# land1725/albedo

Measured on AMD Instinct MI355X. Metric: implicit-ALS interactions/sec per sweep at rank 128 (1/8 GPU); top-30 recs users/sec, higher is better.
Workload: dtype fp32 (split-fp16x3 MFMA build, fp32 accumulate; fp64 Gram/eigenbasis)

## Files before the change

albedo_amd/csrc/als_engine.cpp:

```cpp
#include <hip/hip_runtime.h>
#include <rccl/rccl.h>

#include <algorithm>
#include <chrono>
#include <thread>
#include <cmath>
#include <cstdlib>
#include <functional>
#include <mutex>
#include <cstring>
#include <numeric>
#include <string>
#include <vector>

#include "albedo_als.h"
#include "engine.h"
#include "host_math.h"
#include "kernels.h"

using namespace albedo;

namespace {

thread_local std::string g_err;
// ... 9 lines not shown
#define NCCLCHK(x)                                                                                 \
  do {                                                                                             \
    ncclResult_t r_ = (x);                                                                         \
    if (r_ != ncclSuccess) return fail(ALS_E_RCCL, std::string("RCCL error: ") + ncclGetErrorString(r_) + " in " #x); \
  } while (0)

int albedo::set_device(als_ctx* c) {
  HIPCHK(hipSetDevice(c->dev));
  return ALS_OK;
}

hipError_t albedo::copy_st(const als_ctx* c, void* dst, const void* src, size_t bytes, hipMemcpyKind kind) {
  if (bytes == 0) return hipSuccess;
  const hipError_t e = hipMemcpyAsync(dst, src, bytes, kind, c->st);
  return e != hipSuccess ? e : hipStreamSynchronize(c->st);
}

namespace {

hipError_t fill_st(const als_ctx* c, void* dst, int v, size_t bytes) {
  if (bytes == 0) return hipSuccess;
  const hipError_t e = hipMemsetAsync(dst, v, bytes, c->st);
  return e != hipSuccess ? e : hipStreamSynchronize(c->st);
}

int drain(als_ctx* c) {
  if (c->st2) HIPCHK(hipStreamSynchronize(c->st2));
  if (c->st) HIPCHK(hipStreamSynchronize(c->st));
  return ALS_OK;
}

int validate(const als_params* p) {
  auto bad = [](const char* name, double v) {
    char buf[160];
    snprintf(buf, sizeof buf, "als parameter %s given invalid value %g.", name, v);
    return fail(ALS_E_INVALID_ARGUMENT, buf);
  };
  if (p->rank < 1) return bad("rank", p->rank);
  if (p->max_iter < 0) return bad("maxIter", p->max_iter);
  if (!(p->reg_param >= 0)) return bad("regParam", p->reg_param);
  if (!(p->alpha >= 0)) return bad("alpha", p->alpha);
  if (p->num_user_blocks < 1) return bad("numUserBlocks", p->num_user_blocks);
  if (p->num_item_blocks < 1) return bad("numItemBlocks", p->num_item_blocks);
  if (padded_rank(p->rank) == 0)
    return fail(ALS_E_UNSUPPORTED, "rank " + std::to_string(p->rank) + " exceeds the compiled maximum (256)");
  return ALS_OK;
}

int64_t light_limit(const als_ctx* c) {
  if (c->p.light_max_degree >= 0) return std::min<int64_t>(c->p.light_max_degree, c->KP == 128 ? 96 : 64);
  return c->KP >= 128 ? 64 : 32;
}

int bucket_of(int64_t d, int64_t lmax) {
  if (d <= lmax) {
    if (d <= 16) return B_L16;
    if (d <= 32) return B_L32;
    return d <= 64 ? B_L64 : B_L96;
  }
  return B_HEAVY;
}

int allreduce_G(als_ctx* c) {
  const int64_t n = (int64_t)c->KP * c->KP;
  if (c->world == 1) return ALS_OK;
  if (c->comm) {
    NCCLCHK(ncclAllReduce(c->d_G.p, c->d_G.p, n, ncclDouble, ncclSum, c->comm, c->st));
    return ALS_OK;
  }
  std::vector<double> h(n);
  HIPCHK(hipMemcpyAsync(h.data(), c->d_G.p, n * 8, hipMemcpyDeviceToHost, c->st));
  HIPCHK(hipStreamSynchronize(c->st));
  if (c->h_allreduce(c->h_user, h.data(), n) != 0) return fail(ALS_E_RCCL, "host all-reduce callback failed");
  HIPCHK(hipMemcpyAsync(c->d_G.p, h.data(), n * 8, hipMemcpyHostToDevice, c->st));
  HIPCHK(hipStreamSynchronize(c->st));
  return ALS_OK;
}

int allgather_rows(als_ctx* c, float* buf, int64_t rows_per_rank, hipStream_t s) {
  if (c->world == 1) return ALS_OK;
  const int64_t per = rows_per_rank * c->KP;
  if (c->comm) {
    NCCLCHK(ncclAllGather(buf + (int64_t)c->rank * per, buf, per, ncclFloat, c->comm, s));
    return ALS_OK;
  }
  std::vector<float> h((size_t)per * c->world);
  HIPCHK(hipMemcpyAsync(h.data() + (size_t)c->rank * per, buf + (int64_t)c->rank * per, per * 4,
                        hipMemcpyDeviceToHost, s));
  HIPCHK(hipStreamSynchronize(s));
  if (c->h_allgather(c->h_user, h.data(), per) != 0) return fail(ALS_E_RCCL, "host all-gather callback failed");
  HIPCHK(hipMemcpyAsync(buf, h.data(), h.size() * 4, hipMemcpyHostToDevice, s));
  HIPCHK(hipStreamSynchronize(s));
  return ALS_OK;
}

}

int albedo::allgather_host(als_ctx* c, float* buf, int64_t n) {
  if (c->world == 1) return ALS_OK;
  if (c->comm) {
    DevBuf d;
    HIPCHK(d.ensure((size_t)n * c->world * 4));
    float* dp = d.as<float>();
    HIPCHK(hipMemcpyAsync(dp + (int64_t)c->rank * n, buf + (int64_t)c->rank * n, n * 4, hipMemcpyHostToDevice, c->st));
    NCCLCHK(ncclAllGather(dp + (int64_t)c->rank * n, dp, n, ncclFloat, c->comm, c->st));
    HIPCHK(hipMemcpyAsync(buf, dp, (size_t)n * c->world * 4, hipMemcpyDeviceToHost, c->st));
    HIPCHK(hipStreamSynchronize(c->st));
    return ALS_OK;
  }
  if (c->h_allgather(c->h_user, buf, n) != 0) return fail(ALS_E_RCCL, "host all-gather callback failed");
  return ALS_OK;
}

namespace {

int gather_chunks(als_ctx* c, const Side& S, const float* own, float* full, int q0, int q1, hipStream_t s) {
  const int64_t per = S.chpad * c->KP;
  for (int q = q0; q < q1; ++q) {
    float* base = full + (int64_t)q * c->world * per;
    HIPCHK(hipMemcpyAsync(base + (int64_t)c->rank * per, own + (int64_t)q * per, per * 4, hipMemcpyDeviceToDevice, s));
    TRYC(allgather_rows(c, base, S.chpad, s));
  }
  return ALS_OK;
}

int split_chunk_len() {
  const char* e = std::getenv("ALBEDO_SPLIT_CHUNK");
  if (e && *e) return std::max(0, std::atoi(e));
  return 8192;
}

constexpr int BATCH_SLOTS[5] = {16, 8, 4, 2, 1};
constexpr int BATCH_MIN_SLOTS = 8;
int nnls_min_slots() {
  const char* e = std::getenv("ALBEDO_NNLS_MIN_SLOTS");
  const int v = e && *e ? std::atoi(e) : BATCH_MIN_SLOTS;
  return (v == 16 || v == 8 || v == 4 || v == 2 || v == 1) ? v : BATCH_MIN_SLOTS;
}
int64_t nnls_batch_rows_limit(const als_ctx* c, int v) {
  if (BATCH_SLOTS[v] < nnls_min_slots()) return 0;
  return std::min<int64_t>(nnls_batch_max_degree(c->KP, BATCH_SLOTS[v]), light_limit(c));
}

int gather_chunk_count() { return 4; }

bool use_wave_kernel(const als_ctx* c);

int factor_buffers(als_ctx* c);

int rank_layout(als_ctx* c) {
  TRYC(drain(c));
  const int64_t lmax = light_limit(c);
  c->split_len = split_chunk_len();
  for (int side = 0; side < 2; ++side) {
    Side& S = c->s[side];
    std::vector<int32_t> rows[NBUCKET];
    for (int b = 0; b < NBUCKET; ++b) S.bnnz[b] = 0;
    for (int64_t r = 0; r < S.own_n; ++r) {
      const int b = bucket_of(S.h_deg[r], lmax);
      rows[b].push_back((int32_t)r);
      S.bnnz[b] += S.h_deg[r];
    }
    std::stable_sort(rows[B_HEAVY].begin(), rows[B_HEAVY].end(),
                     [&](int32_t a, int32_t b) { return S.h_deg[a] > S.h_deg[b]; });
    S.n_batch = S.n_batch_nnz = 0;
    for (int v = 0; v < 6; ++v) S.bat_off[v] = 0;
    if (c->p.nonnegative) {
      for (int b = 0; b < B_HEAVY; ++b)
        std::stable_sort(rows[b].begin(), rows[b].end(), [&](int32_t x, int32_t y) { return S.h_deg[x] < S.h_deg[y]; });
      int64_t pos = 0;
      std::vector<int32_t> light;
      for (int b = 0; b < B_HEAVY; ++b) light.insert(light.end(), rows[b].begin(), rows[b].end());
      for (int v = 0; v < 5; ++v) {
        const int64_t dl = nnls_batch_rows_limit(c, v);
        while (pos < (int64_t)light.size() && S.h_deg[light[pos]] <= dl) S.n_batch_nnz += S.h_deg[light[pos++]];
        S.bat_off[v + 1] = pos;
      }
      S.n_batch = pos;
    }
    const int nsolve = (c->world > 1 && !c->p.nonnegative) ? S.nch : 1;
    S.nsolve = nsolve;
    auto chunk_of = [&](int32_t r) { return nsolve == 1 ? 0 : (int)std::min<int64_t>(r / S.chpad, nsolve - 1); };
    std::vector<int32_t> all;
    all.reserve(S.own_n);
    for (int b = 0; b < NBUCKET; ++b) {
      S.boff[b] = (int64_t)all.size();
      const bool pairs = b == B_L16;
      std::stable_sort(rows[b].begin(), rows[b].end(), [&](int32_t x, int32_t y) {
        const int cx = chunk_of(x), cy = chunk_of(y);
        if (cx != cy || !pairs) return cx < cy;
        return (S.h_deg[x] <= 8) > (S.h_deg[y] <= 8);
      });
      int64_t p = 0;
      for (int q = 0; q <= nsolve; ++q) {
        while (q < nsolve && p < (int64_t)rows[b].size() && chunk_of(rows[b][p]) < q) ++p;
        S.cb[b][q] = S.boff[b] + (q == nsolve ? (int64_t)rows[b].size() : p);
      }
      if (pairs)
        for (int q = 0; q < nsolve; ++q) {
          int64_t k = 0;
          for (int64_t i = S.cb[b][q] - S.boff[b]; i < S.cb[b][q + 1] - S.boff[b] && S.h_deg[rows[b][i]] <= 8; ++i) ++k;
          S.c8[q] = k;
        }
      all.insert(all.end(), rows[b].begin(), rows[b].end());
    }
    S.boff[NBUCKET] = (int64_t)all.size();
    HIPCHK(S.d_rows.ensure(all.size() * 4));
    HIPCHK(copy_st(c, S.d_rows.p, all.data(), all.size() * 4, hipMemcpyHostToDevice));
    HIPCHK(S.d_desc.ensure(all.size() * 16));
    HIPCHK(launch_row_desc(S.d_rows.as<int32_t>(), (int64_t)all.size(), S.d_ptr.as<int64_t>(), S.d_desc.as<int32_t>(), c->st));
    HIPCHK(hipStreamSynchronize(c->st));
    const int64_t CH = c->split_len;
// ... 187 lines not shown
  S.orig_valid = false;
  S.full_valid = false;
  return ALS_OK;
}

int spark_init(als_ctx* c) {
  int64_t su, si;
  spark_side_seeds(c->p.seed, &su, &si);
  for (int side = 0; side < 2; ++side) {
    Side& S = c->s[side];
    if (S.has_factors) continue;
    std::vector<float> f((size_t)S.n * c->p.rank);
    spark_initialize(S.ids.data(), S.n, c->p.rank, side == ALS_USER ? su : si,
                     side == ALS_USER ? c->p.num_user_blocks : c->p.num_item_blocks, f.data(), c->p.rank);
    TRYC(upload_factors(c, side, f.data(), c->p.rank));
  }
  return ALS_OK;
}

std::string err_paths(int err) {
  std::string r;
  const std::pair<int, const char*> names[] = {{ALBEDO_EF_LIGHT16, "light16"}, {ALBEDO_EF_LIGHT_REG, "light-d16"},
                                               {ALBEDO_EF_LIGHT_ACC, "light"}, {ALBEDO_EF_WAVE, "wave"},
                                               {ALBEDO_EF_HEAVY, "heavy"}};
  for (const auto& n : names)
    if (err & n.first) r += std::string(r.empty() ? ": " : ",") + n.second;
  return r;
}

}

float albedo::event_ms(hipEvent_t a, hipEvent_t b) {
  float ms = 0.f;
  (void)hipEventElapsedTime(&ms, a, b);
  return ms;
}

namespace {

int column_scales(als_ctx* c, const Side& S, const Side& T, bool have_max = false) {
  const float cmax = c->p.implicit_prefs ? (float)c->p.alpha * T.vmax : 1.0f;
  HIPCHK(launch_colscale(c->KP, S.d_Z.as<float>(), S.prows(), cmax, c->d_csmax.as<unsigned>(),
                         c->d_cs.as<float>(), c->st, have_max));
  return ALS_OK;
}

int heavy_launches(als_ctx* c, const Side& T, SolveArgs a, int64_t h0, int64_t hn, bool nnls, int q = 0);
bool use_wave_kernel(const als_ctx* c);

bool rotate_bf_on(const als_ctx* c) { return c->KP == 128; }

bool presplit_wanted(const als_ctx* c, const Side& T, float* sw) {
  const bool uniform = !c->p.implicit_prefs || (T.vmin == T.vmax && T.vmax > 0.f);
  if (!uniform || !use_wave_kernel(c) || T.boff[NBUCKET] == T.boff[B_HEAVY]) return false;
  const float cw = c->p.implicit_prefs ? (float)c->p.alpha * T.vmax : 1.0f;
  if (!(cw > 0.f)) return false;
  *sw = std::sqrt(cw);
  return true;
}

int presplit(als_ctx* c, const Side& S, const Side& T, const void** zhl, float* wsc, float* inv_sw,
             bool split_done = false) {
  *zhl = nullptr;
  float sw = 1.f;
  if (!presplit_wanted(c, T, &sw)) return ALS_OK;
  const float cw = c->p.implicit_prefs ? (float)c->p.alpha * T.vmax : 1.0f;
  HIPCHK(c->d_Zhl.ensure((size_t)(S.prows() + 1) * c->KP * 4));
  if (!split_done)
    HIPCHK(launch_presplit(c->KP, S.d_Z.as<float>(), S.prows(), c->d_cs.as<float>(), sw, c->d_Zhl.p, c->st));
  const double wmax = c->p.implicit_prefs ? 1.0 + (double)cw : (double)T.vmax;
  int e = 0;
  std::frexp(wmax > 0.0 ? wmax : 1.0, &e);
  *wsc = (float)std::ldexp(1.0, std::max(-60, std::min(60, 13 - e)));
  *inv_sw = 1.0f / sw;
  *zhl = c->d_Zhl.p;
  return ALS_OK;
}

int half_sweep_nnls(als_ctx* c, int t) {
  const int sidx = 1 - t;
  Side& S = c->s[sidx];
  Side& T = c->s[t];
  const int KP = c->KP, k = c->p.rank;
  hipStream_t st = c->st;
  hipEvent_t* ev = c->ev;
  const int ngt = nnls_gtile_floats(KP);
  std::vector<float> gt(ngt, 0.f);
  float gscale = 1.0f;
  if (c->p.implicit_prefs) {
    HIPCHK(launch_gram(KP, S.d_X.as<float>(), S.own_n, c->slab.as<double>(), c->slab_blocks, c->d_G.as<double>(), st));
    TRYC(allreduce_G(c));
    std::vector<double> Gf((size_t)KP * KP);
    HIPCHK(hipMemcpyAsync(Gf.data(), c->d_G.p, Gf.size() * 8, hipMemcpyDeviceToHost, st));
    HIPCHK(hipMemcpyAsync(S.d_Gk.p, c->d_G.p, (size_t)KP * KP * 8, hipMemcpyDeviceToDevice, st));
    HIPCHK(hipMemcpyAsync(S.d_GB.p, S.d_B.p, (size_t)KP * KP * 8, hipMemcpyDeviceToDevice, st));
    HIPCHK(hipStreamSynchronize(st));
    S.has_gram = true;
    for (int i = 0; i < KP; ++i)
      for (int j = 0; j < 16 * ((i >> 4) + 1); ++j) gt[nnls_gtile_index(i, j)] = (float)Gf[(size_t)i * KP + j];
    double gmax = 0.0;
    for (double v : Gf) gmax = std::max(gmax, std::fabs(v));
    if (gmax > 0.0) {
      int ex = 0;
      (void)std::frexp(gmax, &ex);
      gscale = (float)std::ldexp(1.0, std::max(-120, std::min(120, 15 - ex)));
    }
  }
// ... 194 lines not shown
    }
    HIPCHK(hipEventRecord(ev[2], st));
    const float* Xs = multi ? S.d_Xfull.as<float>() : S.d_X.as<float>();
    const int64_t ns = multi ? S.prows() : S.own_n;
    if (rotate_bf_on(c) && !singular) {
      TRYC(column_scales(c, S, T, true));
      cs_done = true;
      float sw = 1.f;
      split_done = presplit_wanted(c, T, &sw);
      if (split_done) HIPCHK(c->d_Zhl.ensure((size_t)(S.prows() + 1) * KP * 4));
      HIPCHK(c->d_Pf.ensure((size_t)rotate_bf_pfrag_bytes(KP)));
      HIPCHK(launch_rotate_bf(KP, Xs, c->d_P.as<float>(), c->d_Pf.p, S.d_Z.as<float>(), ns, c->d_cs.as<float>(), sw,
                              split_done ? c->d_Zhl.p : nullptr, S.prows(), c->n_cu, st));
    } else {
      HIPCHK(hipMemsetAsync(c->d_csmax.p, 0, KP * sizeof(unsigned), st));
      HIPCHK(launch_rotate(KP, Xs, c->d_P.as<float>(), S.d_Z.as<float>(), ns, st, c->d_csmax.as<unsigned>()));
      have_cmax = true;
    }
  } else {
    HIPCHK(hipEventRecord(ev[1], st));
    HIPCHK(hipMemsetAsync(c->d_lam.p, 0, KP * 4, st));
    HIPCHK(hipMemcpyAsync(T.d_B.p, S.d_B.p, (size_t)KP * KP * 8, hipMemcpyDeviceToDevice, st));
    if (c->p.reg_param == 0.0) force_heavy = true;
    HIPCHK(hipEventRecord(ev[2], st));
    if (multi) HIPCHK(hipMemcpyAsync(S.d_Z.p, S.d_Xfull.p, (size_t)S.prows() * KP * 4, hipMemcpyDeviceToDevice, st));
    else HIPCHK(hipMemcpyAsync(S.d_Z.p, S.d_X.p, (size_t)S.own_n * KP * 4, hipMemcpyDeviceToDevice, st));
  }
  HIPCHK(hipEventRecord(ev[3], st));
  if (!cs_done) TRYC(column_scales(c, S, T, have_cmax));
  const void* zhl = nullptr;
  float wsc = 1.f, inv_sw = 1.f;
  TRYC(presplit(c, S, T, &zhl, &wsc, &inv_sw, split_done));
  HIPCHK(hipEventRecord(ev[4], st));
  HIPCHK(hipMemsetAsync(c->d_err.p, 0, 4, st));
  SolveArgs a{};
  a.Zhl = zhl;
  a.zero_row = S.prows();
  a.wsc = wsc;
  a.inv_sw = inv_sw;
  a.Z = S.d_Z.as<float>();
  a.ptr = T.d_ptr.as<int64_t>();
  a.col = T.d_col.as<int32_t>();
  a.val = T.d_val.as<float>();
  a.lam = c->d_lam.as<float>();
  a.X = T.d_X.as<float>();
  a.kreal = k;
  a.implicit = c->p.implicit_prefs;
  a.alpha = (float)c->p.alpha;
  a.reg = (float)c->p.reg_param;
  a.err = c->d_err.as<int>();
  a.colscale = c->d_cs.as<float>();
  a.n_cu = c->n_cu;
  const int32_t* rows = T.d_rows.as<int32_t>();
  static const int Dof[B_HEAVY] = {16, 32, 64, 96};
  T.stats[0] = T.stats[1] = T.stats[2] = T.stats[3] = 0;
  for (int b = 0; b < B_HEAVY; ++b) {
    T.stats[force_heavy ? 2 : 0] += T.boff[b + 1] - T.boff[b];
    T.stats[force_heavy ? 3 : 1] += T.bnnz[b];
  }
  T.stats[2] += T.boff[B_HEAVY + 1] - T.boff[B_HEAVY];
  T.stats[3] += T.bnnz[B_HEAVY];
  for (int q = 0; q < T.nsolve; ++q) {
    for (int b = 0; b < B_HEAVY; ++b) {
      a.rows = rows + T.cb[b][q];
      a.desc = T.d_desc.as<int32_t>() + 4 * T.cb[b][q];
      a.n_rows = T.cb[b][q + 1] - T.cb[b][q];
      if (force_heavy && use_wave_kernel(c)) HIPCHK(launch_solve_wave(KP, a, st));
      else if (force_heavy) HIPCHK(launch_solve_heavy(KP, a, st));
      else if (b == B_L16) {
        SolveArgs p8 = a, p16 = a;
        p8.n_rows = T.c8[q];
        p16.rows += T.c8[q];
        p16.desc += 4 * T.c8[q];
        p16.n_rows -= T.c8[q];
        HIPCHK(launch_solve_light16(KP, p8, st, true));
        HIPCHK(launch_solve_light16(KP, p16, st, false));
      } else HIPCHK(launch_solve_light(KP, Dof[b], a, st));
    }
    if (T.nsolve == 1) HIPCHK(hipEventRecord(ev[5], st));
    TRYC(heavy_launches(c, T, a, T.cb[B_HEAVY][q], T.cb[B_HEAVY][q + 1] - T.cb[B_HEAVY][q], false, q));
    if (multi) {
      HIPCHK(hipEventRecord(c->evc[q], st));
      HIPCHK(hipStreamWaitEvent(c->st2, c->evc[q], 0));
      TRYC(gather_chunks(c, T, T.d_X.as<float>(), T.d_Xfull.as<float>(), q, q + 1, c->st2));
    }
  }
  if (T.nsolve > 1) HIPCHK(hipEventRecord(ev[5], st));
  if (multi) {
    if (T.nsolve == 1) TRYC(gather_chunks(c, T, T.d_X.as<float>(), T.d_Xfull.as<float>(), 0, T.nch, c->st2));
    HIPCHK(hipEventRecord(c->evc[8], c->st2));
  }
  HIPCHK(hipEventRecord(ev[6], st));
  int err = 0, sweeps = 0;
  HIPCHK(hipMemcpyAsync(&err, c->d_err.p, 4, hipMemcpyDeviceToHost, st));
  if (c->p.implicit_prefs) HIPCHK(hipMemcpyAsync(&sweeps, eig_sweeps(c->d_eig.as<double>(), KP), 4, hipMemcpyDeviceToHost, st));
  HIPCHK(hipStreamSynchronize(st));
  T.solver[0] = sweeps == EIG_NOT_FINITE ? 0 : (sweeps < 0 ? -sweeps - 1 : sweeps);
  T.solver[1] = T.solver[2] = T.solver[3] = 0;
  T.t[ALS_T_GRAM] = event_ms(ev[0], ev[1]);
  T.t[ALS_T_EIG] = event_ms(ev[1], ev[2]);
  T.t[ALS_T_ROTATE] = event_ms(ev[2], ev[3]);
  T.t[ALS_T_COMM] = event_ms(ev[3], ev[4]);
  if (T.nsolve > 1) {
    T.t[ALS_T_SOLVE_LIGHT] = 0.0;
    T.t[ALS_T_SOLVE_HEAVY] = event_ms(ev[4], ev[5]);
  } else {
    T.t[ALS_T_SOLVE_LIGHT] = event_ms(ev[4], ev[5]);
    T.t[ALS_T_SOLVE_HEAVY] = event_ms(ev[5], ev[6]);
  }
  T.t[ALS_T_HALF_TOTAL] = event_ms(ev[0], ev[6]);
  if (sweeps == EIG_NOT_FINITE)
    return fail(ALS_E_NOT_POSITIVE_DEFINITE,
                std::string("the ") + (t == ALS_USER ? "item" : "user") +
                    " Gram matrix is not finite (NaN or Inf in the source factors, or row norms past fp32): "
                    "the eigensolver did not converge");
  if (sweeps < 0)
    return fail(ALS_E_NOT_POSITIVE_DEFINITE, "eigensolver did not converge (device Jacobi: " +
                                                 std::to_string(-sweeps - 1) + " sweeps without meeting the tolerance)");
  if (err & 3)
    return fail(ALS_E_NOT_POSITIVE_DEFINITE,
                "LAPACK.dppsv-equivalent Cholesky met a non-positive pivot because A is not positive "
                "definite. Is A derived from a singular matrix (e.g. collinear column values)? (flags " +
                    std::to_string(err) + err_paths(err) + ", " + std::to_string(sweeps) + " eigensolver sweeps, " +
                    (t == ALS_USER ? "user" : "item") + " half)" +
                    failure_diag(c, S, T, c->p.implicit_prefs ? (multi ? S.prows() : S.own_n) : S.own_n, zhl));
  T.has_factors = true;
  T.orig_valid = false;
  T.full_valid = multi;
  return ALS_OK;
}

}
// ... 95 lines not shown
    return fail(ALS_E_HIP, "failed to create a HIP stream");
  }
  for (auto& e : c->ev) (void)hipEventCreate(&e);
  for (auto& e : c->evt) (void)hipEventCreate(&e);
  for (auto& e : c->evc) (void)hipEventCreateWithFlags(&e, hipEventDisableTiming);
  if (hipStreamCreateWithFlags(&c->st2, hipStreamNonBlocking) != hipSuccess) {
    delete c;
    return fail(ALS_E_HIP, "failed to create a HIP stream");
  }
  *out = c;
  return ALS_OK;
}

int als_create(const als_params* p, als_ctx** out) {
  if (!p || !out) return fail(ALS_E_INVALID_ARGUMENT, "null argument");
  *out = nullptr;
  TRYC(validate(p));
  return ctx_common(p, out);
}

int als_set_params(als_ctx* c, const als_params* p) {
  if (!c || !p) return fail(ALS_E_INVALID_ARGUMENT, "null argument");
  if (c->model_only) return fail(ALS_E_STATE, "als_set_params on a model-only context");
  if (c->parent) return fail(ALS_E_STATE, "als_set_params on a fork (fork the parent again instead)");
  {
    std::lock_guard<std::mutex> lk(g_fork_mu);
    if (c->forks > 0) return fail(ALS_E_STATE, "als_set_params while forks view this context's layout");
  }
  TRYC(validate(p));
  TRYC(set_device(c));
  const int dev = c->dev;
  c->p = *p;
  c->p.device = dev;
  c->KP = padded_rank(p->rank);
  if (c->has_ratings) TRYC(rank_layout(c));
  return ALS_OK;
}

int als_fork(als_ctx* parent, const als_params* p, als_ctx** out) {
  if (!parent || !p || !out) return fail(ALS_E_INVALID_ARGUMENT, "null argument");
  *out = nullptr;
  if (!parent->has_ratings || parent->model_only) return fail(ALS_E_STATE, "als_fork needs a context holding ratings");
  if (parent->world > 1) return fail(ALS_E_UNSUPPORTED, "als_fork of a sharded (multi-rank) context");
  TRYC(validate(p));
  if (p->rank != parent->p.rank || p->nonnegative != parent->p.nonnegative ||
      p->light_max_degree != parent->p.light_max_degree)
    return fail(ALS_E_INVALID_ARGUMENT, "a fork keeps its parent's rank, nonnegative and light_max_degree");
  als_params q = *p;
  q.device = parent->dev;
  als_ctx* c = nullptr;
  TRYC(ctx_common(&q, &c));
  c->nnz = parent->nnz;
  c->split_len = parent->split_len;
  for (int side = 0; side < 2; ++side) {
    Side& S = c->s[side];
    const Side& P = parent->s[side];
    S.n = P.n;
    S.ids = P.ids;
    S.starts = P.starts;
    S.maxrows = P.maxrows;
    S.nch = P.nch;
    S.world = P.world;
    S.chpad = P.chpad;
    S.own0 = P.own0;
    S.own_n = P.own_n;
    S.own_nnz = P.own_nnz;
    S.h_deg = P.h_deg;
    S.vmax = P.vmax;
    S.vmin = P.vmin;
    S.d_ptr.share(P.d_ptr);
    S.d_col.share(P.d_col);
    S.d_val.share(P.d_val);
    S.d_rows.share(P.d_rows);
    S.d_desc.share(P.d_desc);
    S.d_chunk_row.share(P.d_chunk_row);
    S.d_chunk_idx.share(P.d_chunk_idx);
    S.d_slot0.share(P.d_slot0);
    std::memcpy(S.boff, P.boff, sizeof S.boff);
    std::memcpy(S.bnnz, P.bnnz, sizeof S.bnnz);
    S.n_split = P.n_split;
    S.n_chunks = P.n_chunks;
    S.n_batch = P.n_batch;
    S.n_batch_nnz = P.n_batch_nnz;
    std::memcpy(S.bat_off, P.bat_off, sizeof S.bat_off);
    S.nsolve = P.nsolve;
    std::memcpy(S.cb, P.cb, sizeof S.cb);
    std::memcpy(S.c8, P.c8, sizeof S.c8);
    std::memcpy(S.split_n, P.split_n, sizeof S.split_n);
    std::memcpy(S.ck_off, P.ck_off, sizeof S.ck_off);
    std::memcpy(S.sl_off, P.sl_off, sizeof S.sl_off);
  }
  {
    std::lock_guard<std::mutex> lk(g_fork_mu);
    ++parent->forks;
  }
  c->parent = parent;
  c->has_ratings = true;
  if (int rc = set_device(c); rc != ALS_OK || (rc = factor_buffers(c)) != ALS_OK) {
    const std::string msg = g_err;
    als_destroy(c);
    return fail(rc, msg);
  }
  *out = c;
  return ALS_OK;
}

// ... 495 lines not shown
```

albedo_amd/csrc/als_kernels.hip:

```cpp
#include <hip/hip_runtime.h>
#include <cmath>
#include <cstdlib>
#include <cstdint>
#include <type_traits>
#include <algorithm>
#include <utility>
#include "kernels.h"
#include "device_common.h"
#include "wave_chol.h"
#include "nnls_common.h"
#include "split_rec.h"

namespace albedo {

inline SolveArgs chunk_args(const SolveArgs& a, int64_t r0, int threads, int rec_floats) {
  SolveArgs b = a;
  b.rows = a.rows + r0;
  b.n_rows = std::min<int64_t>(a.n_rows - r0, max_rows_per_launch(threads));
  if (a.prebuilt) b.prebuilt = a.prebuilt + (size_t)r0 * rec_floats;
  return b;
}

#ifdef ALBEDO_HEAVY_TIMING
__device__ unsigned long long albedo_heavy_ts[64][48];
// ... 489 lines not shown
  f32x4 xa[NK][2], xb[NK][2];
  if (t < ntile) xload(t, xa);
  if (t + tstep < ntile) xload(t + tstep, xb);
  for (; t < ntile; t += 2 * tstep) {
    tile(t, xa, t + 2 * tstep);
    if (t + tstep >= ntile) break;
    tile(t + tstep, xb, t + 3 * tstep);
  }
}

hipError_t launch_rotate_bf(int KP, const float* X, const float* P, void* Pf, float* Z, int64_t n, const float* cs, float sw,
                            void* Zhl, int64_t zrow, int n_cu, hipStream_t s) {
  if (KP != 128) return hipErrorInvalidValue;
  rotate_pfrag_kernel<<<(KP * KP + 255) / 256, 256, 0, s>>>(P, reinterpret_cast<__bf16*>(Pf), KP);
  if (n <= 0) return hipGetLastError();
  const size_t lds = (size_t)KP * KP * 3 * 2 + (size_t)RBF_WAVES * 16 * RBF_TS * 4 + (size_t)KP * 4;
  static const hipError_t attr = allow_lds(rotate_bf_kernel<128>, lds);
  if (attr != hipSuccess) return attr;
  const int64_t tiles = (n + 15) / 16;
  int64_t blocks = (tiles + RBF_WAVES - 1) / RBF_WAVES;
  if (blocks > n_cu) blocks = n_cu;
  rotate_bf_kernel<128><<<(int)blocks, 64 * RBF_WAVES, lds, s>>>(X, reinterpret_cast<const __bf16*>(Pf), Z, n, cs, sw,
                                                                 reinterpret_cast<_Float16*>(Zhl), zrow);
  return hipGetLastError();
}
int rotate_bf_pfrag_bytes(int KP) { return KP * KP * 3 * 2; }

hipError_t launch_rotate(int KP, const float* X, const float* M, float* Z, int64_t n, hipStream_t s, unsigned* cmax) {
  if (n <= 0) return hipSuccess;
  int64_t blocks = (n + 16 * ROT_WAVES - 1) / (16 * ROT_WAVES);
  if (blocks > 1024) blocks = 1024;
  const int nth = 64 * ROT_WAVES;
  if (KP == 64) {
    const size_t lds = (size_t)64 * 68 * 4;
    rotate_kernel<64><<<(int)blocks, nth, lds, s>>>(X, M, Z, n, cmax);
  } else if (KP == 128) {
    const size_t lds = (size_t)128 * 132 * 4;
    static const hipError_t attr = allow_lds(rotate_kernel<128>, lds);
    if (attr != hipSuccess) return attr;
    rotate_kernel<128><<<(int)blocks, nth, lds, s>>>(X, M, Z, n, cmax);
  } else if (KP == 256) {
    const size_t lds = (size_t)256 * (rotate_cols<256>() + 4) * 4;
    static const hipError_t attr = allow_lds(rotate_kernel<256>, lds);
    if (attr != hipSuccess) return attr;
    rotate_kernel<256><<<dim3((int)blocks, 256 / rotate_cols<256>()), nth, lds, s>>>(X, M, Z, n, cmax);
  } else return hipErrorInvalidValue;
  return hipGetLastError();
}

__host__ __device__ constexpr int light_wave_lds(int D) { return D == 16 ? D * (D + 1) / 2 + 64 : wchol_scratch_floats(D / 16); }

template <int KP, int D>
constexpr int light_occupancy() {
  return D > 64 ? 2 : (D == 16 && KP <= 128) ? 6 : (KP == 128 && D == 32) ? 3 : (KP <= 128) ? 4 : 2;
}

template <int KP, int D>
constexpr bool light_keepz() { return D <= 32 && D * KP <= 4096; }
template <int KP, int D>
constexpr bool light_split_s() { return D >= 64 || light_keepz<KP, D>(); }

template <int KP, int D>
__device__ __forceinline__ void light_row(const SolveArgs& a, int j, int d, float r, int colE, float r2, int colE2,
                                          const float (&lamv)[KP / 64], const float (&icsv)[KP / 64], float* smem,
                                          int wave) {
  constexpr int NB = D / 16, NT = NB * (NB + 1) / 2, TRI = light_wave_lds(D), NHC = KP / 64;
  constexpr bool TWO = D > 64;
  const int lane = threadIdx.x & 63, g = lane >> 4, i16 = lane & 15;
  float* Ks = smem + wave * TRI;
  float ce = 0.f, we = 0.f, ce2 = 0.f, we2 = 0.f;
  if (lane < d) rating_weights(r, a.implicit, a.alpha, ce, we);
  if (TWO && 64 + lane < d) rating_weights(r2, a.implicit, a.alpha, ce2, we2);
  const bool valid = lane < d && ce > 0.f;
  const bool valid2 = TWO && 64 + lane < d && ce2 > 0.f;
  const int npos = a.implicit ? __popcll(__ballot(lane < d && r > 0.f)) + (TWO ? __popcll(__ballot(64 + lane < d && r2 > 0.f)) : 0)
                              : d;
  const float lamn = a.reg * (float)npos;

  int colB[NB];
  bool vB[NB];
#pragma unroll
  for (int I = 0; I < NB; ++I) {
    colB[I] = __shfl(I < 4 ? colE : colE2, 16 * (I & 3) + i16);
    vB[I] = __shfl((int)(I < 4 ? valid : valid2), 16 * (I & 3) + i16) != 0;
  }
  constexpr int NC = KP / 16;
  constexpr bool KEEPZ = light_keepz<KP, D>();
  f32x4 zf[KEEPZ ? NB : 1][KEEPZ ? NC : 1];
  if constexpr (KEEPZ) {
#pragma unroll
    for (int I = 0; I < NB; ++I)
#pragma unroll
      for (int c = 0; c < NC; ++c) zf[I][c] = vB[I] ? ld4(a.Z + (int64_t)colB[I] * KP + 16 * c + 4 * g) : zero4();
  }
  constexpr bool PUSHG = !KEEPZ && D >= 64;
  constexpr int LATE = (KP == 128 && D == 64) ? 2 : 0;
  f32x4 zr0[PUSHG ? NB : 1], zr1[PUSHG ? NB : 1];
  const float* zpB[PUSHG ? NB : 1];
  if constexpr (PUSHG) {
#pragma unroll
    for (int I = 0; I < NB; ++I) {
      zpB[I] = a.Z + (vB[I] ? (int64_t)colB[I] : a.zero_row) * KP + 8 * g;
      zr0[I] = ld4(zpB[I]);
      zr1[I] = ld4(zpB[I] + 4);
    }
  }
  f32x4 acc[NT];
#pragma unroll
  for (int t = 0; t < NT; ++t) acc[t] = zero4();
  float* sdl = smem + 4 * TRI + wave * KP;
  bool bad = false;
#pragma unroll
  for (int h = 0; h < NHC; ++h) {
    const int cc = lane + 64 * h;
    const float dd = lamv[h] + lamn;
    if (cc < a.kreal && !(dd > 0.f)) bad = true;
    sdl[cc] = (cc < a.kreal && dd > 0.f) ? frsq(dd) : 0.f;
  }
  WAVE_LDS_SYNC();
  if constexpr (light_split_s<KP, D>()) {
    float bnd = 0.f;
#pragma unroll
    for (int h = 0; h < NHC; ++h) {
      const int cc = lane + 64 * h;
      bnd = fmaxf(bnd, sdl[cc] * icsv[h]);
    }
    bnd = wave_max_dpp(bnd);
    int ex = 0;
    frexpf(bnd * 8192.f, &ex);
    const float sc = ldexpf(1.f, 13 - ex), usc = ldexpf(1.f, 2 * (ex - 13));
    constexpr int NQ = KP / 32;
#pragma unroll
    for (int q = 0; q < NQ; ++q) {
      if constexpr (PUSHG) {
        __builtin_amdgcn_sched_barrier(0);
        if (q > 0) {
#pragma unroll
          for (int I = NB - LATE; I < NB; ++I) {
            zr0[I] = ld4(zpB[I] + 32 * q);
            zr1[I] = ld4(zpB[I] + 32 * q + 4);
          }
          __builtin_amdgcn_sched_barrier(0);
        }
      }
      const f32x4 s0 = KEEPZ ? ld4(sdl + 32 * q + 4 * g) : ld4(sdl + 32 * q + 8 * g);
      const f32x4 s1 = KEEPZ ? ld4(sdl + 32 * q + 16 + 4 * g) : ld4(sdl + 32 * q + 8 * g + 4);
      f16x8 zh[NB], zl[NB];
#pragma unroll
      for (int I = 0; I < NB; ++I) {
// ... 191 lines not shown
    for (int h = 0; h < NHC; ++h) sd[h] = sdl[NHC * lane + h];
    *reinterpret_cast<xvec*>(a.X + (int64_t)j * KP + NHC * lane) = xacc * (sd * sd);
  }
}

template <int KP, int D>
__global__ __launch_bounds__(256, (light_occupancy<KP, D>())) void solve_light_kernel(SolveArgs a) {
  extern __shared__ __attribute__((aligned(16))) float smem[];
  const int lane = threadIdx.x & 63;
  const int wave = __builtin_amdgcn_readfirstlane(threadIdx.x >> 6);
  const int64_t ridx = (int64_t)blockIdx.x * 4 + wave;
  if (ridx >= a.n_rows) return;
  float lamv[KP / 64], icsv[KP / 64];
#pragma unroll
  for (int h = 0; h < KP / 64; ++h) {
    lamv[h] = a.lam[lane + 64 * h];
    icsv[h] = light_split_s<KP, D>() ? a.colscale[KP + lane + 64 * h] : 0.f;
  }
  typedef __attribute__((address_space(4))) const int cint;
  cint* q = (cint*)(a.desc) + 4 * ridx;
  const int j = q[0], d = q[3];
  const int64_t p0 = (int64_t)(uint32_t)q[1] | ((int64_t)q[2] << 32);
  float r = 0.f, r2 = 0.f;
  int colE = 0, colE2 = 0;
  if (lane < d) {
    r = a.val[p0 + lane];
    colE = a.col[p0 + lane];
  }
  if (D > 64 && 64 + lane < d) {
    r2 = a.val[p0 + 64 + lane];
    colE2 = a.col[p0 + 64 + lane];
  }
  light_row<KP, D>(a, j, d, r, colE, r2, colE2, lamv, icsv, smem, wave);
}

hipError_t launch_solve_light(int KP, int D, const SolveArgs& a0, hipStream_t s) {
  if (a0.n_rows <= 0) return hipSuccess;
  if (!a0.desc) return hipErrorInvalidValue;
  if (a0.n_rows > max_rows_per_launch(64)) {
    for (int64_t r0 = 0; r0 < a0.n_rows; r0 += max_rows_per_launch(64)) {
      SolveArgs b = chunk_args(a0, r0, 64, 0);
      b.desc = a0.desc + 4 * r0;
      const hipError_t e = launch_solve_light(KP, D, b, s);
      if (e != hipSuccess) return e;
    }
    return hipSuccess;
  }
  const SolveArgs& a = a0;
  const size_t lds = ((size_t)4 * light_wave_lds(D) + (size_t)4 * KP) * sizeof(float);
  const int blocks = (int)((a.n_rows + 3) / 4);
#define LIGHT(kp, dd) \
  if (KP == kp && D == dd) { solve_light_kernel<kp, dd><<<blocks, 256, lds, s>>>(a); return hipGetLastError(); }
  LIGHT(64, 16) LIGHT(64, 32) LIGHT(64, 64) LIGHT(128, 16) LIGHT(128, 32) LIGHT(128, 64)
  LIGHT(256, 16) LIGHT(256, 32) LIGHT(256, 64) LIGHT(128, 96)
#undef LIGHT
  return hipErrorInvalidValue;
}



template <int KP>
struct Heavy {
  static constexpr int NW = KP >= 256 ? 16 : 4, NTH = 64 * NW, NQ = KP / 16;
  static constexpr int SPS = KP >= 256 ? 64 : 32;
  static constexpr int NU = SPS / 8;
  static constexpr int CS = 2 * SPS;
  static constexpr int IMG = KP * CS;
  static constexpr int NCH = KP / 4, NSG = NTH / NCH, NST = SPS / NSG;
  static constexpr bool PERM = KP != 256;
  static constexpr int SWZ = NU == 4 ? 3 : 5;
  static constexpr int GS = KP == 64 ? 2 : 4, NG = NQ / GS;
  static constexpr int NTL = NQ * (NQ + 1) / 2;
  static constexpr int TILES = NTL * HT_SZ, STAGE = IMG;
  static constexpr int BIG = TILES > STAGE ? TILES : STAGE;
  static constexpr int OFF_B = BIG, OFF_DIAG = OFF_B + KP, OFF_FLAG = OFF_DIAG + KP;
  static constexpr int FLOATS = OFF_FLAG + 4;
  static_assert(NG * NG == NW, "one wave per group pair");
  static_assert(NSG * NCH == NTH && NST * NSG == SPS && (NST == 2 || NST == 4), "stage map");
  static_assert(NSG * KP <= STAGE, "b partials fit into the dead stage");
};

template <int KP>
__device__ __forceinline__ int img_off(int col, int byteoff) {
  using H = Heavy<KP>;
  const int sw = (col ^ (H::SWZ * (col >> 3))) & (H::NU - 1);
  return col * H::CS + ((((byteoff >> 4) ^ sw) & (H::NU - 1)) << 4) + (byteoff & 15);
}

__device__ __forceinline__ uint32_t pack_h2(float a, float b) {
  f16x2 h = {(_Float16)a, (_Float16)b};
  return __builtin_bit_cast(uint32_t, h);
}

template <int KP, bool DIAG, bool NT = false>
__device__ __forceinline__ void heavy_build(const SolveArgs& a, int64_t p0, int d, float* smem, int rb, int cb) {
  using H = Heavy<KP>;
  constexpr int NR = DIAG ? H::GS : H::GS / 2, NC = H::GS, NST = H::NST;
  constexpr int MT = DIAG ? NR * (NR + 1) / 2 : NR * NC;
  const int tid = threadIdx.x, lane = tid & 63, g = lane >> 4, i16 = lane & 15;
  char* lds = reinterpret_cast<char*>(smem);
  int* s_flag = reinterpret_cast<int*>(smem + H::OFF_FLAG);
  const int cc = tid % H::NCH, sg = tid / H::NCH;
  const int xr = H::PERM ? (cc & 3) : 0;
  const f32x4 csc = ld4(a.colscale + 4 * cc);
  f32x4 bp = zero4();
  int npos = 0;
  f32x4 zr[NST];
// ... 1151 lines not shown
```

albedo_amd/csrc/engine.h:

```cpp
#pragma once
#include <hip/hip_runtime.h>
#include <rccl/rccl.h>

#include <cstdint>
#include <string>
#include <vector>

#include "albedo_als.h"

namespace albedo {

int fail(int code, const std::string& msg);

#define HIPCHK(x)                                                                                  \
  do {                                                                                             \
    hipError_t e_ = (x);                                                                           \
    if (e_ != hipSuccess)                                                                          \
      return fail(e_ == hipErrorOutOfMemory ? ALS_E_OUT_OF_MEMORY : ALS_E_HIP,                     \
                  std::string("HIP error: ") + hipGetErrorString(e_) + " in " #x);                 \
  } while (0)
#define TRYC(x)                    \
  do {                             \
    int rc_ = (x);                 \
    if (rc_ != ALS_OK) return rc_; \
// ... 12 lines not shown
    p = nullptr;
    bytes = 0;
    owned = true;
  }
  void share(const DevBuf& o) {
    release();
    p = o.p;
    bytes = o.bytes;
    owned = false;
  }
  hipError_t ensure(size_t b) {
    if (!owned) return hipErrorNotSupported;
    if (b <= bytes && p) return hipSuccess;
    release();
    hipError_t e = hipMalloc(&p, b ? b : 16);
    if (e == hipSuccess) bytes = b;
    return e;
  }
  template <class T>
  T* as() const { return reinterpret_cast<T*>(p); }
};

struct Stream {
  hipStream_t s = nullptr;
  Stream() = default;
  Stream(const Stream&) = delete;
  Stream& operator=(const Stream&) = delete;
  ~Stream() { reset(); }
  bool create() {
    if (hipStreamCreateWithFlags(&s, hipStreamNonBlocking) != hipSuccess) s = nullptr;
    return s != nullptr;
  }
  void reset() {
    if (s) (void)hipStreamDestroy(s);
    s = nullptr;
  }
};
struct Event {
  hipEvent_t e = nullptr;
  Event() = default;
  Event(const Event&) = delete;
  Event& operator=(const Event&) = delete;
  ~Event() { reset(); }
  bool create() {
    if (hipEventCreateWithFlags(&e, hipEventDisableTiming) != hipSuccess) e = nullptr;
    return e != nullptr;
  }
  void reset() {
    if (e) (void)hipEventDestroy(e);
    e = nullptr;
  }
};

enum { B_L16 = 0, B_L32 = 1, B_L64 = 2, B_L96 = 3, B_HEAVY = 4, NBUCKET = 5 };

struct Side {
  int64_t n = 0;
  std::vector<int32_t> ids;
  std::vector<int64_t> starts;
  int64_t maxrows = 0;
  int nch = 1, world = 1;
  int64_t chpad = 0;
  int64_t own0 = 0, own_n = 0;
  DevBuf d_ptr, d_col, d_val;
  int64_t own_nnz = 0;
  std::vector<int64_t> h_deg;
  DevBuf d_rows;
  DevBuf d_desc;
  int64_t boff[NBUCKET + 1] = {0};
  int64_t bnnz[NBUCKET] = {0};
  float vmax = 0.f;
  float vmin = 0.f;
  DevBuf d_X;
  DevBuf d_Z;
  DevBuf d_Xfull;
  bool full_valid = false;
  int64_t prows() const { return (int64_t)nch * world * chpad; }
  int64_t pos(int r, int64_t i) const { return (i / chpad) * world * chpad + (int64_t)r * chpad + i % chpad; }
  DevBuf d_B;
  DevBuf d_Gk;
  DevBuf d_GB;
  bool has_gram = false;
  bool has_factors = false;
  double t[ALS_T_COUNT] = {0};
  int64_t stats[4] = {0};
  int64_t solver[4] = {0};
  DevBuf d_orig;
  bool orig_valid = false;
  int64_t n_split = 0, n_chunks = 0;
  DevBuf d_chunk_row, d_chunk_idx, d_slot0;
  int64_t n_batch = 0, n_batch_nnz = 0;
  int64_t bat_off[6] = {0};
  int nsolve = 1;
  int64_t cb[NBUCKET][9] = {{0}};
  int64_t c8[8] = {0};
  int64_t split_n[8] = {0}, ck_off[9] = {0}, sl_off[8] = {0};
};

}

struct als_ctx {
  using DevBuf = albedo::DevBuf;
  using Side = albedo::Side;
  als_params p{};
  int KP = 0;
  int dev = 0;
  hipStream_t st = nullptr;
  int rank = 0, world = 1;
  ncclComm_t comm = nullptr;
  int (*h_allreduce)(void*, double*, int64_t) = nullptr;
  int (*h_allgather)(void*, float*, int64_t) = nullptr;
  void* h_user = nullptr;
  Side s[2];
  int64_t nnz = 0;
  bool has_ratings = false;
  bool model_only = false;
  DevBuf slab, d_G, d_P, d_lam, d_err, d_Gt, d_cs, d_csmax;
  DevBuf d_eig;
  DevBuf d_partial, d_reduced;
  DevBuf d_Zhl;
  DevBuf d_Pf;
  DevBuf d_iters;
  DevBuf d_gfrag, d_counter;
  int n_cu = 256;
  int64_t topk_stats[4] = {0, 0, 0, 0};
  double topk_ms[5] = {0, 0, 0, 0, 0};
  double eval_ms[5] = {0, 0, 0, 0, 0};
  hipEvent_t evt[5] = {};
  mutable std::vector<int32_t> last_rescan;
  DevBuf d_last_need;
  double* h_plan = nullptr;
  int64_t last_need_n = 0;
  std::vector<int32_t> last_rows;
  mutable bool last_rescan_ready = true;
  bool last_rows_dense = false;
  int last_src = 0;
  int split_len = 0;
  int slab_blocks = 0;
  hipEvent_t ev[8] = {};
  hipStream_t st2 = nullptr;
  als_ctx* parent = nullptr;
  int forks = 0;
  bool doomed = false;
  hipEvent_t evc[9] = {};
};

namespace albedo {

int set_device(als_ctx* c);
hipError_t copy_st(const als_ctx* c, void* dst, const void* src, size_t bytes, hipMemcpyKind kind);
float event_ms(hipEvent_t a, hipEvent_t b);
int materialize(als_ctx* c, int side);
int64_t find_row(const Side& S, int32_t id);
int allgather_host(als_ctx* c, float* buf, int64_t n);

}
```

Measured before the change: 4.605 billion.

## Add degree-48 and degree-80 solve tiers for rank-128 ALS

Adds two new degree buckets at rank 128: a light tier for rows of degree 33-48 and a medium tier for degree 65-80 just above the light limit. Rows in these tiers now go to specialised light-solve kernels with tuned occupancy and prefetch settings instead of padded D=64 or heavy kernels. The aim is to cut wasted padded work, and to move moderately heavy rows off the heavier wave/heavy path. It adds template instantiations and an environment toggle, and changes where the event separating light and heavy work is recorded.

```diff
diff --git a/albedo_amd/csrc/als_engine.cpp b/albedo_amd/csrc/als_engine.cpp
--- a/albedo_amd/csrc/als_engine.cpp
+++ b/albedo_amd/csrc/als_engine.cpp
@@ -85,13 +85,20 @@
   return c->KP >= 128 ? 64 : 32;
 }
 
-int bucket_of(int64_t d, int64_t lmax) {
+bool degree_tiers_on(const als_ctx* c) {
+  if (c->KP != 128 || c->p.light_max_degree != -1 || c->p.nonnegative) return false;
+  const char* e = std::getenv("ALBEDO_DEGREE_TIERS");
+  return !(e && *e && std::atoi(e) == 0);
+}
+
+int bucket_of(int64_t d, int64_t lmax, bool tiers) {
   if (d <= lmax) {
     if (d <= 16) return B_L16;
     if (d <= 32) return B_L32;
+    if (tiers && d <= 48) return B_L48;
     return d <= 64 ? B_L64 : B_L96;
   }
-  return B_HEAVY;
+  return (tiers && d <= 80) ? B_M80 : B_HEAVY;
 }
 
 int allreduce_G(als_ctx* c) {
@@ -185,12 +192,13 @@
   TRYC(drain(c));
   const int64_t lmax = light_limit(c);
   c->split_len = split_chunk_len();
+  c->tiers = degree_tiers_on(c);
   for (int side = 0; side < 2; ++side) {
     Side& S = c->s[side];
     std::vector<int32_t> rows[NBUCKET];
     for (int b = 0; b < NBUCKET; ++b) S.bnnz[b] = 0;
     for (int64_t r = 0; r < S.own_n; ++r) {
-      const int b = bucket_of(S.h_deg[r], lmax);
+      const int b = bucket_of(S.h_deg[r], lmax, c->tiers);
       rows[b].push_back((int32_t)r);
       S.bnnz[b] += S.h_deg[r];
     }
@@ -484,7 +492,7 @@
 
 bool presplit_wanted(const als_ctx* c, const Side& T, float* sw) {
   const bool uniform = !c->p.implicit_prefs || (T.vmin == T.vmax && T.vmax > 0.f);
-  if (!uniform || !use_wave_kernel(c) || T.boff[NBUCKET] == T.boff[B_HEAVY]) return false;
+  if (!uniform || !use_wave_kernel(c) || T.boff[NBUCKET] == T.boff[B_LIGHT_END]) return false;
   const float cw = c->p.implicit_prefs ? (float)c->p.alpha * T.vmax : 1.0f;
   if (!(cw > 0.f)) return false;
   *sw = std::sqrt(cw);
@@ -785,16 +793,19 @@
   a.colscale = c->d_cs.as<float>();
   a.n_cu = c->n_cu;
   const int32_t* rows = T.d_rows.as<int32_t>();
-  static const int Dof[B_HEAVY] = {16, 32, 64, 96};
+  static const int Dof[B_HEAVY] = {16, 32, 48, 64, 96, 80};
   T.stats[0] = T.stats[1] = T.stats[2] = T.stats[3] = 0;
-  for (int b = 0; b < B_HEAVY; ++b) {
+  for (int b = 0; b < B_LIGHT_END; ++b) {
     T.stats[force_heavy ? 2 : 0] += T.boff[b + 1] - T.boff[b];
     T.stats[force_heavy ? 3 : 1] += T.bnnz[b];
   }
-  T.stats[2] += T.boff[B_HEAVY + 1] - T.boff[B_HEAVY];
-  T.stats[3] += T.bnnz[B_HEAVY];
+  for (int b = B_LIGHT_END; b < NBUCKET; ++b) {
+    T.stats[2] += T.boff[b + 1] - T.boff[b];
+    T.stats[3] += T.bnnz[b];
+  }
   for (int q = 0; q < T.nsolve; ++q) {
     for (int b = 0; b < B_HEAVY; ++b) {
+      if (b == B_LIGHT_END && T.nsolve == 1) HIPCHK(hipEventRecord(ev[5], st));
       a.rows = rows + T.cb[b][q];
       a.desc = T.d_desc.as<int32_t>() + 4 * T.cb[b][q];
       a.n_rows = T.cb[b][q + 1] - T.cb[b][q];
@@ -810,7 +821,6 @@
         HIPCHK(launch_solve_light16(KP, p16, st, false));
       } else HIPCHK(launch_solve_light(KP, Dof[b], a, st));
     }
-    if (T.nsolve == 1) HIPCHK(hipEventRecord(ev[5], st));
     TRYC(heavy_launches(c, T, a, T.cb[B_HEAVY][q], T.cb[B_HEAVY][q + 1] - T.cb[B_HEAVY][q], false, q));
     if (multi) {
       HIPCHK(hipEventRecord(c->evc[q], st));
@@ -1012,6 +1022,7 @@
   TRYC(ctx_common(&q, &c));
   c->nnz = parent->nnz;
   c->split_len = parent->split_len;
+  c->tiers = parent->tiers;
   for (int side = 0; side < 2; ++side) {
     Side& S = c->s[side];
     const Side& P = parent->s[side];
diff --git a/albedo_amd/csrc/als_kernels.hip b/albedo_amd/csrc/als_kernels.hip
--- a/albedo_amd/csrc/als_kernels.hip
+++ b/albedo_amd/csrc/als_kernels.hip
@@ -565,13 +565,14 @@
 
 template <int KP, int D>
 constexpr int light_occupancy() {
-  return D > 64 ? 2 : (D == 16 && KP <= 128) ? 6 : (KP == 128 && D == 32) ? 3 : (KP <= 128) ? 4 : 2;
+  return (KP == 128 && D == 80) ? 3 : (KP == 128 && D == 48) ? 5 : D > 64 ? 2 : (D == 16 && KP <= 128) ? 6 :
+         (KP == 128 && D == 32) ? 3 : (KP <= 128) ? 4 : 2;
 }
 
 template <int KP, int D>
 constexpr bool light_keepz() { return D <= 32 && D * KP <= 4096; }
 template <int KP, int D>
-constexpr bool light_split_s() { return D >= 64 || light_keepz<KP, D>(); }
+constexpr bool light_split_s() { return D >= 48 || light_keepz<KP, D>(); }
 
 template <int KP, int D>
 __device__ __forceinline__ void light_row(const SolveArgs& a, int j, int d, float r, int colE, float r2, int colE2,
@@ -606,8 +607,8 @@
 #pragma unroll
       for (int c = 0; c < NC; ++c) zf[I][c] = vB[I] ? ld4(a.Z + (int64_t)colB[I] * KP + 16 * c + 4 * g) : zero4();
   }
-  constexpr bool PUSHG = !KEEPZ && D >= 64;
-  constexpr int LATE = (KP == 128 && D == 64) ? 2 : 0;
+  constexpr bool PUSHG = !KEEPZ && D >= 48;
+  constexpr int LATE = (KP == 128 && D == 64) ? 2 : (KP == 128 && D == 80) ? 3 : 0;
   f32x4 zr0[PUSHG ? NB : 1], zr1[PUSHG ? NB : 1];
   const float* zpB[PUSHG ? NB : 1];
   if constexpr (PUSHG) {
@@ -905,7 +906,7 @@
 #define LIGHT(kp, dd) \
   if (KP == kp && D == dd) { solve_light_kernel<kp, dd><<<blocks, 256, lds, s>>>(a); return hipGetLastError(); }
   LIGHT(64, 16) LIGHT(64, 32) LIGHT(64, 64) LIGHT(128, 16) LIGHT(128, 32) LIGHT(128, 64)
-  LIGHT(256, 16) LIGHT(256, 32) LIGHT(256, 64) LIGHT(128, 96)
+  LIGHT(256, 16) LIGHT(256, 32) LIGHT(256, 64) LIGHT(128, 96) LIGHT(128, 48) LIGHT(128, 80)
 #undef LIGHT
   return hipErrorInvalidValue;
 }
diff --git a/albedo_amd/csrc/engine.h b/albedo_amd/csrc/engine.h
--- a/albedo_amd/csrc/engine.h
+++ b/albedo_amd/csrc/engine.h
@@ -88,7 +88,7 @@
   }
 };
 
-enum { B_L16 = 0, B_L32 = 1, B_L64 = 2, B_L96 = 3, B_HEAVY = 4, NBUCKET = 5 };
+enum { B_L16 = 0, B_L32 = 1, B_L48 = 2, B_L64 = 3, B_L96 = 4, B_M80 = 5, B_HEAVY = 6, NBUCKET = 7, B_LIGHT_END = B_M80 };
 
 struct Side {
   int64_t n = 0;
@@ -172,6 +172,7 @@
   bool last_rows_dense = false;
   int last_src = 0;
   int split_len = 0;
+  bool tiers = false;
   int slab_blocks = 0;
   hipEvent_t ev[8] = {};
   hipStream_t st2 = nullptr;
```

Result: faster. 4.703 billion, median of 6 (+2.1%).
